# richarddurbin/modimizer

Hardware: AMD Instinct MI355X
Metric: Gbp/s hashed+sketched (k=21,d=64) (higher is better)
Workload: dtype u64; 1 GPU; BASELINE config 2: 10 Gbp synthetic ONT-like reads (log-normal N50 20 kb, 5% subs, 30x of a 333 Mbp genome), k=21 d=64 seed=17, seqhash scan + modset build (table bits 30); reads_per_gpu=598835, bases_per_gpu=10000000000, modimizers_per_gpu=156043826, modset_entries=102967436, k=21, d=64, table_bits=30, parallelism=reads sharded x1, modset per GPU

## Files before the change

modimizer_amd/csrc/mg_common.h:

```cpp
#ifndef MG_COMMON_H
#define MG_COMMON_H
#include "mg_knobs.h"

#include <hip/hip_runtime.h>
#include <stdint.h>
#include <time.h>
#include <algorithm>
#include <vector>
#include "modgpu.h"

#define MG_WAVE 64

#define MG_SCAN_THREADS   256
#define MG_POS_PER_THREAD 64
#define MG_TILE_BASES     (64 * MG_POS_PER_THREAD)
#define MG_TILE_WORDS     (MG_TILE_BASES / 16)

struct MgHashParams {
  U64 factor1;
  U64 mask;
  int k;
  int shift1;
  U32 d;
  int dShift;
// ... 110 lines not shown
#define MG_MIX_MUL 0x9E3779B1u
__device__ __forceinline__ U64 mgMixK (U64 x, int b)
{
  if (b < 24) return mgMixBits (x, b);
  const int lb = b - MG_MIX_TOP;
  const U64 L = x & (((U64) 1 << lb) - 1), A = x >> lb;
  const U32 low = lb >= 32 ? (U32) L : ((U32) L & (((U32) 1 << lb) - 1));
  const U32 g = (low * MG_MIX_MUL) >> (32 - MG_MIX_TOP);
  return ((A ^ (U64) g) << lb) | mgMixBits (L, lb);
}
__device__ __forceinline__ U32 mgMixTopOfKmer (U64 x, int b, int hiB)
{
  const int lb = b - MG_MIX_TOP;
  const U32 low = lb >= 32 ? (U32) x : ((U32) x & (((U32) 1 << lb) - 1));
  return (U32) (x >> (b - hiB)) ^ ((low * MG_MIX_MUL) >> (32 - hiB));
}
__device__ __forceinline__ U32 mgBucketOfM (U64 m, const MgGeom &g)
{
  if (!g.log2NB) return 0u;
  const int s = g.kbits - g.log2NB;
  return s >= 0 ? (U32) (m >> s) : ((U32) m << (-s));
}
__device__ __forceinline__ U32 mgHomeOfM (U64 m, const MgGeom &g)
{
  U32 x = (U32) m;
  if (g.kbits >= 24) x ^= (U32) (m >> (g.kbits - MG_MIX_TOP)) * 0x9E5u;
  return __umulhi (x * 0x85EBCA6Bu, g.R);
}
__device__ __forceinline__ U32 mgNextSlot (U32 at, U32 R) { return at + 1 == R ? 0u : at + 1; }
#endif

static inline unsigned mgGrid (U64 n, unsigned per = 256, unsigned cap = 4096)
{ U64 b = (n + per - 1) / per; if (b > cap) b = cap; if (b < 1) b = 1; return (unsigned) b; }
static inline size_t mgAl256 (size_t n) { return (n + 255) & ~(size_t) 255; }
static inline double mgNowS (void) { struct timespec ts; clock_gettime (CLOCK_MONOTONIC, &ts); return ts.tv_sec + 1e-9 * ts.tv_nsec; }

static inline void mgPartSplit (int log2NB, int *hiB, int *loB)
{ if (log2NB <= 9) { *hiB = log2NB; *loB = 0; } else { *loB = log2NB / 2; *hiB = log2NB - *loB; } }

#define MG_HIST_STRIDE 16
struct MgHistReq { int log2NB; int kbits; U32 *binCount; int hiB; };

struct MgSegSrc { const U64 *segKmer; const U64 *segCount; const U64 *segStart; U64 segCap; U32 nSegs; };


MgStatus mgLaunchPack (const U8 *dBases, U64 nBases, U32 *dWords, hipStream_t st);
MgStatus mgLaunchUnpack (const U32 *dWords, U64 nBases, U8 *dBases, hipStream_t st);
MgStatus mgLaunchScan (const MgHashParams &p, const U32 *dPacked, U64 totalBases,
                       const U64 *dReadOffsets, U32 nReads,
                       U64 *dKmer, U32 *dPosF, U32 *dReadId, U64 capacity,
                       U64 *dCount, void *dWork, hipStream_t st, const MgHistReq *hist = 0, MgSegSrc *lazy = 0);

U64      mgScanTiles (U64 totalBases);
size_t   mgScanInfoBytes (U64 totalBases);
MgStatus mgScanPrepare (const U64 *dReadOffsets, U32 nReads, U64 totalBases, void *dInfo, hipStream_t st);
size_t   mgScanRangeWorkBytes (U64 nTilesRange, U64 capacity);
MgStatus mgLaunchSegCompact (const MgSegSrc &src, U64 *dKmer, U64 capacity, const U64 *dCount, hipStream_t st);
MgStatus mgLaunchScanRange (const MgHashParams &p, const U32 *dPacked, U64 totalBases,
                            const U64 *dReadOffsets, U32 nReads, const void *dInfo, U64 tile0, U64 tile1,
                            U64 *dKmer, U32 *dPosF, U32 *dReadId, U64 capacity,
                            U64 *dCount, void *dWork, hipStream_t st, const MgHistReq *hist = 0, MgSegSrc *lazy = 0);

U64      mgIterMaxBases (void);
U64      mgIterSegEntries (void);
MgStatus mgLaunchIterScan (const MgHashParams &p, const U32 *dPacked, U64 totalBases, const U64 *dReadOff,
                           U64 *dSegKmer, U32 *dSegPosF, U64 *out, U64 capEntries, U64 *flag, U64 seq, hipStream_t st);

MgStatus mgLaunchMinimizers (const MgHashParams &p, U32 w, const U32 *dPacked, const U64 *dReadOffsets, U32 nReads,
                             U64 *dHash, U32 *dPosF, U64 *dReadStart, U64 capacity, U64 *totalOut, hipStream_t st);

struct MgSlot { U64 key; U32 ord; U32 cnt; };
struct MgTable {
  MgSlot *slots; U64 nSlots;
  U64 capSlots;
  U32 capNB;
  U32 R; int log2NB;
  int kbits;
  U32 *occ;
  U64 *value;
  U16 *baseDepth;
  bool baseZero;
  U64 *liveHist;
  bool liveHistValid;
  U32 size;
  U32 max;
  U32 syncedMax;
  U64 *counters;
  bool pendingDepth;
  bool dirty;
  U64 *find8;
  U64 find8Cap;
  U64 find8Version, version;
  bool empty;
  U64 *pin;
  int newPct;
  int loadPct;
  int  maxLog2Slots;
  U32  wantR;
  U64  diag[7];
  int  tightPct;
};
MgStatus mgTableAlloc (MgTable *t, U64 slotsWanted, hipStream_t st);
MgStatus mgTableEnsure (MgTable *t, U64 nIncoming, hipStream_t st);
MgStatus mgTableRollback (MgTable *t, hipStream_t st);
MgStatus mgTableClean (MgTable *t, hipStream_t st);
void     mgTableForget (MgTable *t, hipStream_t st);
size_t   mgTableAddScratchBytes (const MgTable *t, U64 n);
bool     mgTableUseBuckets (const MgTable *t, U64 n);
struct MgValueAside { hipStream_t stream; hipEvent_t merged, done; bool launched; };
MgStatus mgTableAdd (MgTable *t, const U64 *dKmer, U64 n, int withDepth, void *scratch, hipStream_t st,
                     const MgHistReq *counted = 0,
                     const MgSegSrc *segSrc = 0,
// ... 31 lines not shown
```

modimizer_amd/csrc/mg_scan.hip:

```cpp
#include <stdlib.h>
#include <atomic>
#include "mg_prefix.h"


__global__ void mgPackKernel (const U8 *__restrict__ bases, U64 nBases, U32 *__restrict__ words, U64 nWords)
{
  U64 i = (U64) blockIdx.x * blockDim.x + threadIdx.x;
  U64 stride = (U64) gridDim.x * blockDim.x;
  const bool aligned = (((uintptr_t) bases) & 15) == 0;
  for ( ; i < nWords ; i += stride)
    { U64 b0 = i * 16;
      U32 w = 0;
      if (b0 + 16 <= nBases && aligned)
        { uint4 v = *reinterpret_cast<const uint4 *> (bases + b0);
          U32 q[4] = { v.x, v.y, v.z, v.w };
#pragma unroll
          for (int j = 0 ; j < 4 ; ++j)
            { U32 x = q[j];
              U32 n = ((x & 3) << 6) | (((x >> 8) & 3) << 4) | (((x >> 16) & 3) << 2) | ((x >> 24) & 3);
              w |= n << (24 - 8 * j);
            }
        }
      else if (b0 < nBases)
        { for (int j = 0 ; j < 16 && b0 + j < nBases ; ++j)
            w |= (U32) (bases[b0 + j] & 3) << (30 - 2 * j);
        }
      words[i] = w;
    }
}

__global__ void mgUnpackKernel (const U32 *__restrict__ words, U64 nBases, U8 *__restrict__ bases)
{
  U64 i = (U64) blockIdx.x * blockDim.x + threadIdx.x;
  U64 stride = (U64) gridDim.x * blockDim.x;
  for ( ; i < nBases ; i += stride)
    bases[i] = (U8) ((words[i >> 4] >> (30 - 2 * (i & 15))) & 3);
}

MgStatus mgLaunchPack (const U8 *dBases, U64 nBases, U32 *dWords, hipStream_t st)
{
  U64 nWords = (U64) mgPackedWords (nBases);
  if (!nWords) return MG_OK;
  U64 blocks = (nWords + 255) / 256; if (blocks > 8192) blocks = 8192;
  MG_LAUNCH (MG_K_PACK, st, mgPackKernel, dim3 ((unsigned) blocks), dim3 (256), 0, st, dBases, nBases, dWords, nWords);
  MG_HIP (hipGetLastError ());
  return MG_OK;
}

MgStatus mgLaunchUnpack (const U32 *dWords, U64 nBases, U8 *dBases, hipStream_t st)
{
  if (!nBases) return MG_OK;
  U64 blocks = (nBases + 255) / 256; if (blocks > 16384) blocks = 16384;
  MG_LAUNCH (MG_K_UNPACK, st, mgUnpackKernel, dim3 ((unsigned) blocks), dim3 (256), 0, st, dWords, nBases, dBases);
  MG_HIP (hipGetLastError ());
  return MG_OK;
}


__device__ __forceinline__ U32 mgReadOf (const U64 *__restrict__ off, U32 lo, U32 hi, U64 p)
{
  while (lo < hi)
    { U32 mid = lo + (hi - lo + 1) / 2;
      if (off[mid] <= p) lo = mid; else hi = mid - 1;
    }
  return lo;
}

struct __attribute__ ((aligned (32))) MgTileInfo { U64 start, end; U32 firstRead, pad0; U64 pad1; };

__global__ void mgTileInfoKernel (const U64 *__restrict__ readOff, U32 nReads, U64 nTiles, U64 totalBases,
                                  MgTileInfo *__restrict__ info)
{
  U64 t = (U64) blockIdx.x * blockDim.x + threadIdx.x;
  if (t > nTiles) return;
  MgTileInfo ti;
  ti.pad0 = 0; ti.pad1 = 0;
  if (t == nTiles) { ti.firstRead = nReads - 1; ti.start = readOff[nReads - 1]; ti.end = totalBases; }
  else
    { U32 r = mgReadOf (readOff, 0, nReads - 1, t * (U64) MG_TILE_BASES);
      ti.firstRead = r; ti.start = readOff[r]; ti.end = readOff[r + 1];
    }
  info[t] = ti;
}


struct MgScanArgs {
  MgHashParams p;
  const U32 *packed; U64 nWordsAlloc; U64 totalBases;
  const U64 *readOff; U32 nReads;
  const MgTileInfo *tileInfo;
  U64 tileBegin, tileLimit;
  U64 tilesPerWorker;
  U64 nWorkers;
  U64 segCap;
  U64 *segKmer; U32 *segPosF; U32 *segRead;
  U64 *blockCount;
  U32 fS, thresh;
  U32 *histCount;
  int histKbits, histHiB;
#ifdef MG_ABLATE
  U32 debug;
#endif
};

__device__ __forceinline__ U64 mgValidMask (const U64 *off, U32 rBase, U32 nReads, int k, U64 p0, U32 rFirst)
{
  U64 valid = 0;
  U32 r = rFirst;
  for (;;)
    { int64_t start = (int64_t) off[r - rBase], end = (int64_t) off[r + 1 - rBase];
      int64_t lo = start > (int64_t) p0 ? start : (int64_t) p0;
      int64_t hi = end - k; if (hi > (int64_t) p0 + 63) hi = (int64_t) p0 + 63;
      if (hi >= lo)
        { int n = (int) (hi - lo + 1);
          U64 m = (n == 64) ? ~0ull : (((1ull << n) - 1) << (int) (lo - (int64_t) p0));
          valid |= m;
        }
      if (end >= (int64_t) p0 + 64 || r + 1 >= nReads) break;
      ++r;
    }
  return valid;
}

__device__ __forceinline__ bool mgTileInside (const MgScanArgs &a, U64 tile) { return (tile + 1) * MG_TILE_WORDS + 8 <= a.nWordsAlloc; }
__device__ __forceinline__ uint4 mgLoadTileWords (const MgScanArgs &a, U64 tile, int tid, bool inside)
{
  U64 g = tile * MG_TILE_WORDS + 4 * (U64) tid;
  uint4 v;
  if (inside || g + 4 <= a.nWordsAlloc) v = *reinterpret_cast<const uint4 *> (a.packed + g);
  else
    { v.x = g     < a.nWordsAlloc ? a.packed[g]     : 0;
      v.y = g + 1 < a.nWordsAlloc ? a.packed[g + 1] : 0;
      v.z = g + 2 < a.nWordsAlloc ? a.packed[g + 2] : 0;
      v.w = 0;
    }
  return v;
}
__device__ __forceinline__ U32 mgLoadTileHalo (const MgScanArgs &a, U64 tile, int lane, bool inside)
{
  U32 h = 0;
  if (lane < 8) { const U64 gh = tile * MG_TILE_WORDS + MG_TILE_WORDS + lane; h = (inside || gh < a.nWordsAlloc) ? a.packed[gh] : 0; }
  return h;
}

__device__ __forceinline__ U64 mgKmerAt (const U32 *sWords, U32 q, int sh1)
{
  int wi = q >> 4, s = 2 * (q & 15);
  U32 x0 = sWords[wi], x1 = sWords[wi + 1], x2 = sWords[wi + 2];
  U64 hi = ((U64) x0 << 32) | x1;
  if (s) hi = (hi << s) | (U64) (x2 >> (32 - s));
  return hi >> sh1;
}

#define MG_MODE_ANY   0
#define MG_MODE_POW2  1
#define MG_MODE_FAST  2
#define MG_MODE_ODD   3
#define MG_MODE_ODD32 4
#define MG_MODE_ANY32 5
#define MG_MODE_COUNT 6
#define MG_LIST_UNROLL 4
#define MG_CAND_CAP   320
#define MG_WAVES      (MG_SCAN_THREADS / 64)
#ifdef MG_ABLATE
#define MG_ABLATE_AND(x) && (x)
#else
#define MG_ABLATE_AND(x)
#endif

#define MG_WAVE_SYNC() do { __builtin_amdgcn_fence (__ATOMIC_RELEASE, "wavefront"); __builtin_amdgcn_wave_barrier (); \
                            __builtin_amdgcn_fence (__ATOMIC_ACQUIRE, "wavefront"); } while (0)

__device__ __forceinline__ void mgScanHistDone (const MgScanArgs &a, U32 *sHist, U32 *sDone, int lane)
{
  U32 before = 0;
  if (lane == 0) before = __hip_atomic_fetch_add (sDone, 1u, __ATOMIC_RELEASE, __HIP_MEMORY_SCOPE_WORKGROUP);
  before = (U32) __builtin_amdgcn_readfirstlane ((int) before);
  if (before != MG_WAVES - 1) return;
  __builtin_amdgcn_fence (__ATOMIC_ACQUIRE, "workgroup");
  const U32 bins = (U32) 1 << a.histHiB;
  for (U32 b = (U32) lane ; b < bins ; b += 64) { const U32 v = sHist[b]; if (v) atomicAdd (&a.histCount[b * MG_HIST_STRIDE], v); }
}

template <int MODE, bool SINGLE, bool WHERE>
__device__ __forceinline__ U64 mgScanWorker (const MgScanArgs &a, const U64 worker, const int lane,
                                             U32 (*sWordsW)[MG_TILE_WORDS + 8], unsigned short *sCand, U64 *sOff, U32 *sHist)
{
  const MgHashParams &p = a.p;
  const int k = p.k, sh1 = p.shift1;
  const U64 f1 = p.factor1;
  const U64 dMask = (U64) (p.d - 1);

  U64 tile = a.tileBegin + worker * a.tilesPerWorker;
  U64 tileEnd = tile + a.tilesPerWorker; if (tileEnd > a.tileLimit) tileEnd = a.tileLimit;
  const U64 segBase = worker * a.segCap;
  U32 found = 0;
  const U32 segCap32 = a.segCap > 0xffffffffull ? 0xffffffffu : (U32) a.segCap;
  U64 *const segK = a.segKmer + segBase;
  uint4 curV = make_uint4 (0, 0, 0, 0); U32 curHalo = 0;
  MgTileInfo ti, tiNext;
  ti.start = ti.end = 0; ti.firstRead = 0; tiNext = ti;
  U32 nextFirstRead = 0;
  if (tile < tileEnd)
    { const bool inside = mgTileInside (a, tile);
      curV = mgLoadTileWords (a, tile, lane, inside);
      curHalo = mgLoadTileHalo (a, tile, lane, inside);
      if (SINGLE) { ti.start = 0; ti.end = a.totalBases; ti.firstRead = 0; }
      else { ti = a.tileInfo[tile]; nextFirstRead = a.tileInfo[tile + 1].firstRead; }
    }

  int buf = 0;
  U32 qCount = 0, qOld = 0;
  while (tile < tileEnd)
    { U32 *sWords = sWordsW[buf]; buf ^= 1;
      *reinterpret_cast<uint4 *> (&sWords[4 * lane]) = curV;
      if (lane < 8) sWords[MG_TILE_WORDS + lane] = curHalo;

      const U64 tile0 = tile * (U64) MG_TILE_BASES;
      const U64 p0 = tile0 + (U64) lane * MG_POS_PER_THREAD;
      U64 valid = 0;
      U32 rFirst = ti.firstRead;
      const bool oneRead = ti.end >= tile0 + MG_TILE_BASES + (U64) k - 1;
      const bool offInLds = !oneRead && nextFirstRead - ti.firstRead + 2 <= 64;
      if (offInLds)
        { const U32 r = ti.firstRead + (U32) lane;
          if (SINGLE) sOff[lane] = lane == 0 ? 0ull : (lane == 1 ? a.totalBases : ~0ull);
          else sOff[lane] = r <= a.nReads ? a.readOff[r] : ~0ull;
        }
      MG_WAVE_SYNC ();
      if (oneRead) valid = ~0ull;
      else if (p0 < a.totalBases)
        { if (offInLds)
            { rFirst = ti.firstRead + mgReadOf (sOff, 0, nextFirstRead - ti.firstRead, p0);
              valid = mgValidMask (sOff, ti.firstRead, a.nReads, k, p0, rFirst);
            }
          else
            { rFirst = mgReadOf (a.readOff, ti.firstRead, nextFirstRead, p0);
              valid = mgValidMask (a.readOff, 0, a.nReads, k, p0, rFirst);
            }
        }

      const U64 nextTile = tile + 1;
      uint4 nextV = make_uint4 (0, 0, 0, 0); U32 nextHalo = 0; U32 nextNextFirst = 0;
      if (nextTile < tileEnd)
        { const bool inside = mgTileInside (a, nextTile);
          nextV = mgLoadTileWords (a, nextTile, lane, inside);
          nextHalo = mgLoadTileHalo (a, nextTile, lane, inside);
          if (SINGLE) tiNext = ti;
          else { tiNext = a.tileInfo[nextTile]; nextNextFirst = a.tileInfo[nextTile + 1].firstRead; }
        }

      U32 w[6];
      { uint2 h = *reinterpret_cast<const uint2 *> (&sWords[4 * lane + 4]);
        w[0] = curV.x; w[1] = curV.y; w[2] = curV.z; w[3] = curV.w; w[4] = h.x; w[5] = h.y;
      }
      U64 cand;
      if (MODE == MG_MODE_FAST)
        {
          U32 fw[6], rw[6];
          const int c2 = 2 * (k - 16);
#pragma unroll
          for (int j = 0 ; j < 5 ; ++j) fw[j] = __builtin_amdgcn_alignbit (w[j], w[j + 1], 32 - c2);
          fw[5] = w[5] << c2;
#pragma unroll
          for (int j = 0 ; j < 6 ; ++j) rw[j] = mgRevComp16 (w[j]);
          const U32 fS = a.fS, thresh = a.thresh;
          U32 acc = 0, candLo = 0;
#pragma unroll
          for (int chunk = 0 ; chunk < 4 ; ++chunk)
            { const U32 f0 = fw[0], f1w = fw[1], r0 = rw[0], r1 = rw[1];
              fw[0] = fw[1]; fw[1] = fw[2]; fw[2] = fw[3]; fw[3] = fw[4]; fw[4] = fw[5];
              rw[0] = rw[1]; rw[1] = rw[2]; rw[2] = rw[3]; rw[3] = rw[4]; rw[4] = rw[5];
#pragma unroll
              for (int tt = 0 ; tt < 16 ; ++tt)
                { U32 xf = __funnelshift_l (f1w, f0, 2 * tt);
                  U32 xr = __funnelshift_r (r0, r1, 2 * tt);
                  U32 hf = xf * fS, hr = xr * fS;
                  U32 mn = hf < hr ? hf : hr;
                  asm ("v_cmp_gt_u32_e32 vcc, %1, %2\n\tv_addc_co_u32_e32 %0, vcc, %0, %0, vcc"
                       : "+v" (acc) : "s" (thresh), "v" (mn) : "vcc");
                }
              if (chunk == 1) { candLo = acc; acc = 0; }
            }
          cand = ((U64) __brev (acc) << 32) | __brev (candLo);
        }
      else
        {
          U32 rw[6];
#pragma unroll
          for (int j = 0 ; j < 6 ; ++j) rw[j] = mgRevComp16 (w[j]);
          const U32 maskLo = (U32) p.mask, maskHi = (U32) (p.mask >> 32);
          U32 acc = 0, hitLo = 0;
#pragma unroll 1
          for (int chunk = 0 ; chunk < 4 ; ++chunk)
            { const U32 f0 = w[0], f1w = w[1], f2 = w[2], r0 = rw[0], r1 = rw[1], r2 = rw[2];
              w[0] = w[1]; w[1] = w[2]; w[2] = w[3]; w[3] = w[4]; w[4] = w[5];
              rw[0] = rw[1]; rw[1] = rw[2]; rw[2] = rw[3]; rw[3] = rw[4]; rw[4] = rw[5];
#pragma unroll
              for (int tt = 0 ; tt < 16 ; ++tt)
                { const U32 wHi = tt ? __builtin_amdgcn_alignbit (f0, f1w, 32 - 2 * tt) : f0;
                  const U32 wLo = tt ? __builtin_amdgcn_alignbit (f1w, f2, 32 - 2 * tt) : f1w;
                  const U32 xLo = tt ? __builtin_amdgcn_alignbit (r1, r0, 2 * tt) : r0;
                  const U32 xHi = tt ? __builtin_amdgcn_alignbit (r2, r1, 2 * tt) : r1;
                  const U64 F = (((U64) wHi << 32) | wLo) >> sh1;
                  const U64 R = ((U64) (xHi & maskHi) << 32) | (xLo & maskLo);
                  U64 hF = (F * f1) >> sh1, hR = (R * f1) >> sh1;
                  U64 h = hF < hR ? hF : hR;
                  bool hit;
                  if (MODE == MG_MODE_POW2)     hit = (h & dMask) == 0;
                  else if (MODE == MG_MODE_ODD) hit = mgDivisibleOdd (h, p);
                  else if (MODE == MG_MODE_ODD32) hit = mgDivisibleOdd32 (h, p);
                  else if (MODE == MG_MODE_ANY32) hit = mgDivisibleAny32 (h, p);
                  else                          hit = mgDivisible (h, p);
                  acc = (acc << 1) | (hit ? 1u : 0u);
                }
              if (chunk == 1) { hitLo = acc; acc = 0; }
            }
          cand = ((U64) __brev (acc) << 32) | __brev (hitLo);
        }
      cand &= valid;

      const U32 cntLo = (U32) __popc ((U32) cand);
      const U32 cnt = cntLo + (U32) __popc ((U32) (cand >> 32));
      const U32 incl = mgWaveInclusiveSum (cnt);
      const U32 nc = (U32) __builtin_amdgcn_readlane ((int) incl, 63);
      const U32 myFirst = incl - cnt;
#ifdef MG_ABLATE
      if (a.debug & 1)
        { tile = nextTile; curV = nextV; curHalo = nextHalo; ti = tiNext; nextFirstRead = nextNextFirst;
          found += nc >> 20;
          continue;
        }
#endif
      constexpr bool wantWhere = WHERE;
      constexpr int LIST_UNROLL = WHERE ? 0 : MG_LIST_UNROLL;
      const bool lastTile = nextTile >= tileEnd;
      const U32 bufTag = (U32) (buf ^ 1) << 12;
      U32 listed = 0;
      do
        { const U32 room = MG_CAND_CAP - qCount;
          const U32 take = nc - listed < room ? nc - listed : room;
          const U32 lo = listed, hi = listed + take;
          if (lo == 0 && hi == nc)
            { unsigned short *pp = sCand + qCount + myFirst;
#pragma unroll
              for (int half = 0 ; half < 2 ; ++half)
                { U32 c = half ? (U32) (cand >> 32) : (U32) cand;
                  const U32 base = bufTag | ((U32) lane * MG_POS_PER_THREAD + 32u * half);
#pragma unroll
                  for (int j = 0 ; j < LIST_UNROLL ; ++j)
                    { if (!c) break;
                      pp[j] = (unsigned short) (base | (U32) __builtin_ctz (c));
                      c &= c - 1;
                    }
                  if (c)
                    { unsigned short *qq = pp + LIST_UNROLL;
                      do { *qq++ = (unsigned short) (base | (U32) __builtin_ctz (c)); c &= c - 1; } while (c);
                    }
                  if (!half) pp += cntLo;
                }
            }
          else if (take && myFirst < hi && myFirst + cnt > lo)
            { U32 o = myFirst - lo;
#pragma unroll
              for (int half = 0 ; half < 2 ; ++half)
                { U32 c = half ? (U32) (cand >> 32) : (U32) cand;
                  const U32 base = bufTag | ((U32) lane * MG_POS_PER_THREAD + 32u * half);
                  while (c)
                    { const U32 t = (U32) __builtin_ctz (c);
                      c &= c - 1;
                      sCand[o < take ? qCount + o : MG_CAND_CAP] = (unsigned short) (base | t);
                      ++o;
                    }
                }
            }
          MG_WAVE_SYNC ();
          qCount += take; listed = hi;
          U32 nEval = qCount & ~63u;
          if (listed == nc && (wantWhere || lastTile || qOld > nEval)) nEval = qCount;
          U32 waveRun = 0;
#pragma unroll 1
          for (U32 i0 = 0 ; i0 < nEval ; i0 += 64)
            { const U32 i = i0 + (U32) lane;
              const U32 e = sCand[i];
              const U32 q = e & (MG_TILE_BASES - 1);
              U64 F = mgKmerAt (sWordsW[(e >> 12) & 1], q, sh1);
              bool surv, fwd;
              { const U64 R = mgRevComp (F, sh1);
                if (MODE == MG_MODE_FAST)
                  {
                    const U64 PF = F * f1, PR = R * f1;
                    const U32 keep = ~((1u << sh1) - 1u);
                    const U64 cF = (PF & 0xffffffff00000000ull) | ((U32) PF & keep), cR = (PR & 0xffffffff00000000ull) | ((U32) PR & keep);
                    fwd = cF < cR;
                    const U32 lowWord = (U32) (fwd ? PF : PR);
                    surv = (lowWord & ((U32) dMask << sh1)) == 0;
                  }
                else
                  { U64 hF = (F * f1) >> sh1, hR = (R * f1) >> sh1;
                    fwd = hF < hR;
                    U64 h = fwd ? hF : hR;
                    if (MODE == MG_MODE_POW2)     surv = (h & dMask) == 0;
                    else if (MODE == MG_MODE_ODD) surv = mgDivisibleOdd (h, p);
                    else if (MODE == MG_MODE_ODD32) surv = mgDivisibleOdd32 (h, p);
                    else if (MODE == MG_MODE_ANY32) surv = mgDivisibleAny32 (h, p);
                    else                          surv = mgDivisible (h, p);
                  }
                if (!fwd) F = R;
              }
              surv = surv && i < nEval MG_ABLATE_AND (!(a.debug & 4));
              const U64 bs = __ballot (surv);
              U32 r = 0;
              if (wantWhere && (!oneRead || a.segRead)) r = (U32) __shfl ((int) rFirst, (int) (q >> 6));
              if (surv)
                { const U32 o = found + waveRun + (U32) __popcll (bs & (((U64) 1 << lane) - 1));
                  const U64 pos = tile0 + q;
                  U64 rs = ti.start;
                  if (!oneRead && wantWhere)
                    { if (offInLds) { while (sOff[r + 1 - ti.firstRead] <= pos) ++r; rs = sOff[r - ti.firstRead]; }
                      else { while (a.readOff[r + 1] <= pos) ++r; rs = a.readOff[r]; }
                    }
                  if (a.histCount) atomicAdd (&sHist[mgMixTopOfKmer (F, a.histKbits, a.histHiB)], 1u);
                  if (o < segCap32 MG_ABLATE_AND (!(a.debug & 2)))
                    { segK[o] = F;
                      if (WHERE && a.segPosF) a.segPosF[segBase + o] = (U32) (pos - rs) | (fwd ? MG_FWD_BIT : 0u);
                      if (WHERE && a.segRead) a.segRead[segBase + o] = r;
                    }
                }
              waveRun += (U32) __popcll (bs);
            }
          found += waveRun;
          const U32 rem = qCount - nEval;
          if (rem && nEval)
            { const U32 v = (U32) lane < rem ? sCand[nEval + lane] : 0u;
              MG_WAVE_SYNC ();
              if ((U32) lane < rem) sCand[lane] = (unsigned short) v;
            }
          if (nEval) MG_WAVE_SYNC ();
          qOld = qOld > nEval ? qOld - nEval : 0;
          qCount = rem;
        }
      while (listed < nc);
      qOld = qCount;
      tile = nextTile;
      curV = nextV; curHalo = nextHalo; ti = tiNext; nextFirstRead = nextNextFirst;
    }
  return found;
}

template <int MODE, bool WHERE>
__global__ __launch_bounds__ (MG_SCAN_THREADS)
void mgScanKernel (const MgScanArgs a)
{
  __shared__ __attribute__ ((aligned (16))) U32 sWordsAll[MG_WAVES][2][MG_TILE_WORDS + 8];
  __shared__ unsigned short sCandAll[MG_WAVES][MG_CAND_CAP + 2];
  __shared__ U64 sOffAll[MG_WAVES][64];
  __shared__ U32 sHist[512]; __shared__ U32 sDone;

  const int lane = threadIdx.x & 63;
  const int wave = __builtin_amdgcn_readfirstlane ((int) (threadIdx.x >> 6));
  const U64 worker = (U64) blockIdx.x * MG_WAVES + wave;
  if (a.histCount)
    { for (U32 b = threadIdx.x ; b < 512 ; b += MG_SCAN_THREADS) sHist[b] = 0;
      if (threadIdx.x == 0) sDone = 0;
      __syncthreads ();
    }
  if (worker >= a.nWorkers) { if (a.histCount) mgScanHistDone (a, sHist, &sDone, lane); return; }
  const U64 found = mgScanWorker<MODE, false, WHERE> (a, worker, lane, sWordsAll[wave], sCandAll[wave], sOffAll[wave], sHist);
  if (lane == 0) a.blockCount[worker] = found;
  if (a.histCount) mgScanHistDone (a, sHist, &sDone, lane);
}

#define MG_ITER_WAVES     8
#define MG_ITER_MAX_TILES 64
struct MgIterOut { U64 *out; U64 capEntries; volatile U64 *flag; U64 seq; };

template <int MODE>
__global__ __launch_bounds__ (MG_ITER_WAVES * 64)
void mgIterScanKernel (const MgScanArgs a, const MgIterOut o)
{
  __shared__ __attribute__ ((aligned (16))) U32 sWordsAll[MG_ITER_WAVES][2][MG_TILE_WORDS + 8];
  __shared__ unsigned short sCandAll[MG_ITER_WAVES][MG_CAND_CAP + 2];
  __shared__ U64 sOffAll[MG_ITER_WAVES][64];
  __shared__ U64 sFound[MG_ITER_WAVES];
  const int lane = threadIdx.x & 63;
  const int wave = __builtin_amdgcn_readfirstlane ((int) (threadIdx.x >> 6));
  U64 found = 0;
  if ((U64) wave < a.nWorkers) found = mgScanWorker<MODE, true, true> (a, (U64) wave, lane, sWordsAll[wave], sCandAll[wave], sOffAll[wave], (U32 *) 0);
  if (lane == 0) sFound[wave] = found;
  __syncthreads ();
  U64 before = 0, total = 0;
#pragma unroll
  for (int w = 0 ; w < MG_ITER_WAVES ; ++w) { const U64 v = sFound[w]; if (w < wave) before += v; total += v; }
  if (total <= o.capEntries)
    { U32 *posOut = reinterpret_cast<U32 *> (o.out + 1 + total);
      const U64 src = (U64) wave * a.segCap;
      for (U64 i = (U64) lane ; i < found ; i += 64)
        { o.out[1 + before + i] = a.segKmer[src + i];
          posOut[before + i] = a.segPosF[src + i];
        }
    }
  if (threadIdx.x == 0) o.out[0] = total;
  __threadfence_system ();
  __syncthreads ();
  if (threadIdx.x == 0) __hip_atomic_store (const_cast<U64 *> (o.flag), o.seq, __ATOMIC_RELEASE, __HIP_MEMORY_SCOPE_SYSTEM);
}

__global__ __launch_bounds__ (1024)
void mgSegScanKernel (const U64 *__restrict__ blockCount, U32 nBlocks, U64 segCap, U64 capacity,
                      U64 *__restrict__ segStart, U64 *__restrict__ dCount)
{
  __shared__ U64 sV[8192 + 1024];
  __shared__ U64 sWaveSum[16], sWaveMax[16];
  const int tid = threadIdx.x, lane = tid & 63, wave = tid >> 6;
  U64 carry = 0, gmx = 0;
  for (U32 base = 0 ; base < nBlocks ; base += 8192)
    {
#pragma unroll
      for (int j = 0 ; j < 8 ; ++j)
        { U32 e = (U32) j * 1024 + tid, b = base + e;
          sV[e + (e >> 3)] = b < nBlocks ? blockCount[b] : 0;
        }
      __syncthreads ();
      U64 c[8], sum = 0, mx = 0;
// ... 68 lines not shown
          for (int j = 0 ; j < 4 ; ++j)
            { const U64 i = i0 + (U64) j * 256 + threadIdx.x;
              if (i >= n) continue;
              if (outKmer) outKmer[dst + i] = km[j];
              if (outPosF) outPosF[dst + i] = pf[j];
              if (outRead) outRead[dst + i] = rd[j];
              if (histBins)
                { MgGeom hg; hg.R = 0; hg.log2NB = histLog2NB; hg.kbits = histKbits;
                  const U32 bucket = mgBucketOfM (mgMixK (km[j], histKbits), hg);
                  atomicAdd (&sH[(bucket >> histShift) & (histBins - 1)], 1u);
                }
            }
        }
    }
  if (histBins)
    { __syncthreads ();
      for (U32 b = threadIdx.x ; b < histBins ; b += 256) if (sH[b]) atomicAdd (&histCount[b * MG_HIST_STRIDE], sH[b]);
    }
}


static inline U64 mgNumTiles (U64 totalBases) { return (totalBases + MG_TILE_BASES - 1) / MG_TILE_BASES; }

struct MgScanGeom { U64 nTiles, tilesPerBlock; U32 nBlocks; U64 segCap; };
#define MG_SCAN_MAX_BLOCKS 49152

static MgScanGeom mgScanGeometryTiles (U64 nTiles, U64 capacity)
{
  MgScanGeom g;
  g.nTiles = nTiles;
  const long gridKnob = mgKnobs ()->scanGrid;
  const long maxBlocks = gridKnob != MG_KNOB_UNSET && gridKnob > 0 ? gridKnob : MG_SCAN_MAX_BLOCKS;
  U64 want = g.nTiles < (U64) maxBlocks ? g.nTiles : (U64) maxBlocks;
  if (gridKnob == MG_KNOB_UNSET || gridKnob <= 0)
    { U64 fewer = g.nTiles / 8; if (fewer < 8192) fewer = 8192;
      if (want > fewer) want = fewer;
    }
  if (!want) want = 1;
  g.tilesPerBlock = (g.nTiles + want - 1) / want; if (!g.tilesPerBlock) g.tilesPerBlock = 1;
  g.nBlocks = (U32) ((g.nTiles + g.tilesPerBlock - 1) / g.tilesPerBlock); if (!g.nBlocks) g.nBlocks = 1;
  U64 share = capacity / g.nBlocks;
  const long slackKnob = mgKnobs ()->segSlack;
  const bool dense = capacity > (g.nTiles * (U64) MG_TILE_BASES) / 16;
  const U64 slack = slackKnob != MG_KNOB_UNSET && slackKnob >= 1 && slackKnob <= 8 ? (U64) slackKnob : 3;
  U64 seg = slack > 1 ? slack * share + 64 : share + share / 8 + 64;
  if (dense && (slackKnob == MG_KNOB_UNSET || slackKnob < 1 || slackKnob > 8)) seg = share + share / 2 + 64;
  U64 most = g.tilesPerBlock * (U64) MG_TILE_BASES;
  g.segCap = seg < most ? seg : most;
  return g;
}


U64 mgScanTiles (U64 totalBases) { return mgNumTiles (totalBases); }
size_t mgScanInfoBytes (U64 totalBases) { return mgAl256 ((mgNumTiles (totalBases) + 2) * sizeof (MgTileInfo)); }

MgStatus mgScanPrepare (const U64 *dReadOffsets, U32 nReads, U64 totalBases, void *dInfo, hipStream_t st)
{
  U64 nTiles = mgNumTiles (totalBases);
  if (!nTiles || !nReads) return MG_OK;
  MG_LAUNCH (MG_K_TILE_FIRST_READ, st, mgTileInfoKernel, dim3 ((unsigned) ((nTiles + 1 + 255) / 256)), dim3 (256), 0, st,
             dReadOffsets, nReads, nTiles, totalBases, (MgTileInfo *) dInfo);
  MG_HIP (hipGetLastError ());
  return MG_OK;
}

size_t mgScanRangeWorkBytes (U64 nTilesRange, U64 capacity)
{
  MgScanGeom g = mgScanGeometryTiles (nTilesRange, capacity);
  size_t segN = (size_t) g.nBlocks * g.segCap;
  return mgAl256 (g.nBlocks * 8) + mgAl256 ((g.nBlocks + 1) * 8) + mgAl256 (segN * 8) + 2 * mgAl256 (segN * 4) + 256;
}

size_t mgScanWorkBytes (U64 totalBases, U32 nReads, U64 capacity)
{
  (void) nReads;
  return mgScanRangeWorkBytes (mgNumTiles (totalBases), capacity) + mgScanInfoBytes (totalBases);
}

static std::atomic<U64> gScanLaunches[3 * MG_MODE_COUNT];
#define MG_SCAN_COUNTED(i) gScanLaunches[i].fetch_add (1, std::memory_order_relaxed)

extern "C" MgStatus mgScanDiag (U64 *out18)
{
  for (int i = 0 ; i < 3 * MG_MODE_COUNT ; ++i) out18[i] = gScanLaunches[i].load (std::memory_order_relaxed);
  return MG_OK;
}

static int mgScanMode (const MgHashParams &p, MgScanArgs *a)
{
  const bool pow2 = (p.dOddInv == 1 && p.dOddLim == ~0ull);
  const int B = p.shift1 + p.dShift;
  const int forceGeneric = mgKnobs ()->scanGeneric == 1;
  a->fS = 0; a->thresh = 0;
  if (pow2 && p.dShift >= 3 && B <= 32 && p.k >= 17 && !forceGeneric)
    { a->fS = (U32) (p.factor1 << (32 - B));
      a->thresh = (U32) 1 << (32 - p.dShift);
      return MG_MODE_FAST;
    }
  if (pow2) return MG_MODE_POW2;
  const bool small = p.small32 && mgKnobs ()->scanDiv64 != 1;
  return p.dShift == 0 ? (small ? MG_MODE_ODD32 : MG_MODE_ODD) : (small ? MG_MODE_ANY32 : MG_MODE_ANY);
}

MgStatus mgLaunchScanRange (const MgHashParams &p, const U32 *dPacked, U64 totalBases,
                            const U64 *dReadOffsets, U32 nReads, const void *dInfo, U64 tile0, U64 tile1,
                            U64 *dKmer, U32 *dPosF, U32 *dReadId, U64 capacity,
                            U64 *dCount, void *dWork, hipStream_t st, const MgHistReq *hist, MgSegSrc *lazy)
{
  if (lazy) { lazy->segKmer = 0; lazy->nSegs = 0; }
  MG_HIP (hipMemsetAsync (dCount, 0, 4 * sizeof (U64), st));
  if (hist && hist->binCount) MG_HIP (hipMemsetAsync (hist->binCount, 0, 512 * MG_HIST_STRIDE * sizeof (U32), st));
  if (tile1 <= tile0 || !nReads) return MG_OK;
  MgScanGeom g = mgScanGeometryTiles (tile1 - tile0, capacity);
  char *wb = (char *) dWork;
  size_t segN = (size_t) g.nBlocks * g.segCap;
  U64 *blockCount = (U64 *) wb;                  wb += mgAl256 (g.nBlocks * 8);
  U64 *segStart = (U64 *) wb;                    wb += mgAl256 ((g.nBlocks + 1) * 8);
  U64 *segKmer = (U64 *) wb;                     wb += mgAl256 (segN * 8);
  U32 *segPosF = (U32 *) wb;                     wb += mgAl256 (segN * 4);
  U32 *segRead = (U32 *) wb;

  MgScanArgs a;
  a.p = p; a.packed = dPacked; a.nWordsAlloc = (U64) mgPackedWords (totalBases); a.totalBases = totalBases;
  a.readOff = dReadOffsets; a.nReads = nReads; a.tileInfo = (const MgTileInfo *) dInfo;
  a.tileBegin = tile0; a.tileLimit = tile1;
  a.tilesPerWorker = g.tilesPerBlock; a.nWorkers = g.nBlocks; a.segCap = g.segCap;
  a.segKmer = segKmer; a.segPosF = dPosF ? segPosF : 0; a.segRead = dReadId ? segRead : 0; a.blockCount = blockCount;
  a.fS = 0; a.thresh = 0;
  int hHiB = 0, hLoB = 0;
  if (hist && hist->binCount)
    { mgPartSplit (hist->log2NB, &hHiB, &hLoB);
      if (hist->hiB > 0 && hist->hiB <= hist->log2NB && hist->hiB <= 9) { hHiB = hist->hiB; hLoB = hist->log2NB - hHiB; }
    }
  const int histEnv = mgKnobs ()->scanHist == 0 ? 0 : 1;
  const bool scanCounts = histEnv && hist && hist->binCount && hist->kbits >= 24 && hHiB >= 1 && hHiB <= MG_MIX_TOP && hLoB + hHiB == hist->log2NB;
  a.histCount = scanCounts ? hist->binCount : 0; a.histKbits = hist ? hist->kbits : 64; a.histHiB = hHiB;
#ifdef MG_ABLATE
  { const long dbg = mgKnobs ()->scanDebug; a.debug = dbg != MG_KNOB_UNSET ? (U32) dbg : 0u; }
#endif
  const unsigned grid = (g.nBlocks + MG_WAVES - 1) / MG_WAVES;
  const int mode = mgScanMode (p, &a);
  const bool where = a.segPosF || a.segRead;
#define MG_SCAN_LAUNCH(M) do { if (where) { MG_SCAN_COUNTED (2 * (M) + 1); MG_LAUNCH (MG_K_SCAN, st, (mgScanKernel<M, true>), dim3 (grid), dim3 (MG_SCAN_THREADS), 0, st, a); } \
                               else       { MG_SCAN_COUNTED (2 * (M));     MG_LAUNCH (MG_K_SCAN, st, (mgScanKernel<M, false>), dim3 (grid), dim3 (MG_SCAN_THREADS), 0, st, a); } } while (0)
  if (mode == MG_MODE_FAST) MG_SCAN_LAUNCH (MG_MODE_FAST); else if (mode == MG_MODE_POW2) MG_SCAN_LAUNCH (MG_MODE_POW2);
  else if (mode == MG_MODE_ODD) MG_SCAN_LAUNCH (MG_MODE_ODD); else if (mode == MG_MODE_ODD32) MG_SCAN_LAUNCH (MG_MODE_ODD32);
  else if (mode == MG_MODE_ANY32) MG_SCAN_LAUNCH (MG_MODE_ANY32); else MG_SCAN_LAUNCH (MG_MODE_ANY);
#undef MG_SCAN_LAUNCH
  MG_HIP (hipGetLastError ());
  MG_LAUNCH (MG_K_SEG_SCAN, st, mgSegScanKernel, dim3 (1), dim3 (1024), 0, st, blockCount, g.nBlocks, g.segCap, capacity, segStart, dCount);
  MG_HIP (hipGetLastError ());
  { int hiB = 0, loB = 0; U32 bins = 0;
    if (hist && hist->binCount && !scanCounts) { mgPartSplit (hist->log2NB, &hiB, &loB); bins = (U32) 1 << hiB; }
    const unsigned cgrid = g.nBlocks < 4096 ? g.nBlocks : 4096;
    if (lazy) { lazy->segKmer = segKmer; lazy->segCount = blockCount; lazy->segStart = segStart; lazy->segCap = g.segCap; lazy->nSegs = g.nBlocks; }
    if (!lazy || bins || dPosF || dReadId)
      MG_LAUNCH (MG_K_SEG_COMPACT, st, mgSegCompactKernel, dim3 (cgrid), dim3 (256), 0, st,
                 segKmer, a.segPosF, a.segRead, g.segCap, g.nBlocks, blockCount, segStart, lazy ? (U64 *) 0 : dKmer, dPosF, dReadId, capacity, dCount,
                 hist ? hist->log2NB : 0, hist ? hist->kbits : 64, loB, bins, hist ? hist->binCount : (U32 *) 0);
  }
  MG_HIP (hipGetLastError ());
  return MG_OK;
}

MgStatus mgLaunchSegCompact (const MgSegSrc &src, U64 *dKmer, U64 capacity, const U64 *dCount, hipStream_t st)
{
  if (!src.nSegs) return MG_OK;
  const unsigned cgrid = src.nSegs < 4096 ? src.nSegs : 4096;
  MG_LAUNCH (MG_K_SEG_COMPACT, st, mgSegCompactKernel, dim3 (cgrid), dim3 (256), 0, st,
             src.segKmer, (const U32 *) 0, (const U32 *) 0, src.segCap, src.nSegs, src.segCount, src.segStart, dKmer, (U32 *) 0, (U32 *) 0, capacity, dCount,
             0, 64, 0, 0u, (U32 *) 0);
  MG_HIP (hipGetLastError ());
  return MG_OK;
}

MgStatus mgLaunchScan (const MgHashParams &p, const U32 *dPacked, U64 totalBases,
                       const U64 *dReadOffsets, U32 nReads,
                       U64 *dKmer, U32 *dPosF, U32 *dReadId, U64 capacity,
                       U64 *dCount, void *dWork, hipStream_t st, const MgHistReq *hist, MgSegSrc *lazy)
{
  const U64 nTiles = mgNumTiles (totalBases);
  char *info = (char *) dWork + mgScanRangeWorkBytes (nTiles, capacity);
  MgStatus s = mgScanPrepare (dReadOffsets, nReads, totalBases, info, st); if (s) return s;
  return mgLaunchScanRange (p, dPacked, totalBases, dReadOffsets, nReads, info, 0, nTiles,
                            dKmer, dPosF, dReadId, capacity, dCount, dWork, st, hist, lazy);
}


U64 mgIterMaxBases (void) { return (U64) MG_ITER_MAX_TILES * MG_TILE_BASES; }
U64 mgIterSegEntries (void) { return (U64) MG_ITER_MAX_TILES * MG_TILE_BASES; }

MgStatus mgLaunchIterScan (const MgHashParams &p, const U32 *dPacked, U64 totalBases, const U64 *dReadOff,
                           U64 *dSegKmer, U32 *dSegPosF, U64 *out, U64 capEntries, U64 *flag, U64 seq, hipStream_t st)
{
  const U64 nTiles = mgNumTiles (totalBases);
  if (!nTiles || nTiles > MG_ITER_MAX_TILES) { mgSetError ("internal: iterator scan of %llu bases", (unsigned long long) totalBases); return MG_ERR_ARG; }
  MgScanArgs a;
  a.p = p; a.packed = dPacked; a.nWordsAlloc = (U64) mgPackedWords (totalBases); a.totalBases = totalBases;
  a.readOff = dReadOff; a.nReads = 1; a.tileInfo = 0;
  a.tileBegin = 0; a.tileLimit = nTiles;
  a.tilesPerWorker = (nTiles + MG_ITER_WAVES - 1) / MG_ITER_WAVES;
  a.nWorkers = (nTiles + a.tilesPerWorker - 1) / a.tilesPerWorker;
  a.segCap = a.tilesPerWorker * (U64) MG_TILE_BASES;
  a.segKmer = dSegKmer; a.segPosF = dSegPosF; a.segRead = 0; a.blockCount = 0;
  a.histCount = 0; a.histKbits = 64; a.histHiB = 0;
#ifdef MG_ABLATE
  a.debug = 0;
#endif
  MgIterOut o; o.out = out; o.capEntries = capEntries; o.flag = flag; o.seq = seq;
  const int mode = mgScanMode (p, &a);
#define MG_ITER_LAUNCH(M) do { MG_SCAN_COUNTED (2 * MG_MODE_COUNT + (M)); hipLaunchKernelGGL (mgIterScanKernel<M>, dim3 (1), dim3 (MG_ITER_WAVES * 64), 0, st, a, o); } while (0)
  if (mode == MG_MODE_FAST) MG_ITER_LAUNCH (MG_MODE_FAST); else if (mode == MG_MODE_POW2) MG_ITER_LAUNCH (MG_MODE_POW2);
  else if (mode == MG_MODE_ODD) MG_ITER_LAUNCH (MG_MODE_ODD); else if (mode == MG_MODE_ODD32) MG_ITER_LAUNCH (MG_MODE_ODD32);
  else if (mode == MG_MODE_ANY32) MG_ITER_LAUNCH (MG_MODE_ANY32); else MG_ITER_LAUNCH (MG_MODE_ANY);
#undef MG_ITER_LAUNCH
  MG_HIP (hipGetLastError ());
  return MG_OK;
}
```

Baseline: 1268 Gbp/s.

## Drop tile-info precompute kernel; locate reads in-scan with wave-parallel search

Removes the separate per-tile read-info kernel and its work buffer. The scan worker now finds the first read of its tile with a wave-cooperative 64-way search and carries read bounds from tile to tile using the offsets already staged in LDS. It also reads some fields directly from the kernarg segment and tunes SGPR limits per specialization to reduce register pressure. This trades one kernel launch and a global table for extra ballots and searches inside the scan loop, and it relies on positions fitting in 32 bits for read starts.

```diff
diff --git a/modimizer_amd/csrc/mg_common.h b/modimizer_amd/csrc/mg_common.h
--- a/modimizer_amd/csrc/mg_common.h
+++ b/modimizer_amd/csrc/mg_common.h
@@ -186,12 +186,10 @@
                        U64 *dCount, void *dWork, hipStream_t st, const MgHistReq *hist = 0, MgSegSrc *lazy = 0);
 
 U64      mgScanTiles (U64 totalBases);
-size_t   mgScanInfoBytes (U64 totalBases);
-MgStatus mgScanPrepare (const U64 *dReadOffsets, U32 nReads, U64 totalBases, void *dInfo, hipStream_t st);
 size_t   mgScanRangeWorkBytes (U64 nTilesRange, U64 capacity);
 MgStatus mgLaunchSegCompact (const MgSegSrc &src, U64 *dKmer, U64 capacity, const U64 *dCount, hipStream_t st);
 MgStatus mgLaunchScanRange (const MgHashParams &p, const U32 *dPacked, U64 totalBases,
-                            const U64 *dReadOffsets, U32 nReads, const void *dInfo, U64 tile0, U64 tile1,
+                            const U64 *dReadOffsets, U32 nReads, U64 tile0, U64 tile1,
                             U64 *dKmer, U32 *dPosF, U32 *dReadId, U64 capacity,
                             U64 *dCount, void *dWork, hipStream_t st, const MgHistReq *hist = 0, MgSegSrc *lazy = 0);
 
diff --git a/modimizer_amd/csrc/mg_scan.hip b/modimizer_amd/csrc/mg_scan.hip
--- a/modimizer_amd/csrc/mg_scan.hip
+++ b/modimizer_amd/csrc/mg_scan.hip
@@ -1,4 +1,5 @@
 #include <stdlib.h>
+#include <stddef.h>
 #include <atomic>
 #include "mg_prefix.h"
 
@@ -66,21 +67,17 @@
   return lo;
 }
 
-struct __attribute__ ((aligned (32))) MgTileInfo { U64 start, end; U32 firstRead, pad0; U64 pad1; };
-
-__global__ void mgTileInfoKernel (const U64 *__restrict__ readOff, U32 nReads, U64 nTiles, U64 totalBases,
-                                  MgTileInfo *__restrict__ info)
-{
-  U64 t = (U64) blockIdx.x * blockDim.x + threadIdx.x;
-  if (t > nTiles) return;
-  MgTileInfo ti;
-  ti.pad0 = 0; ti.pad1 = 0;
-  if (t == nTiles) { ti.firstRead = nReads - 1; ti.start = readOff[nReads - 1]; ti.end = totalBases; }
-  else
-    { U32 r = mgReadOf (readOff, 0, nReads - 1, t * (U64) MG_TILE_BASES);
-      ti.firstRead = r; ti.start = readOff[r]; ti.end = readOff[r + 1];
-    }
-  info[t] = ti;
+__device__ __forceinline__ U32 mgWaveReadOf (const U64 *__restrict__ off, U32 lo, U32 hi, U64 p, int lane)
+{
+  while (lo < hi)
+    { const U32 step = ((hi - lo - 1) >> 6) + 1;
+      const U64 idx = (U64) lo + (U64) (lane + 1) * step;
+      const bool le = idx <= (U64) hi && off[idx] <= p;
+      const U32 c = (U32) __popcll (__ballot (le));
+      lo += c * step;
+      if (hi - lo > step - 1) hi = lo + (step - 1);
+    }
+  return lo;
 }
 
 
@@ -88,7 +85,6 @@
   MgHashParams p;
   const U32 *packed; U64 nWordsAlloc; U64 totalBases;
   const U64 *readOff; U32 nReads;
-  const MgTileInfo *tileInfo;
   U64 tileBegin, tileLimit;
   U64 tilesPerWorker;
   U64 nWorkers;
@@ -171,6 +167,13 @@
 #define MG_WAVE_SYNC() do { __builtin_amdgcn_fence (__ATOMIC_RELEASE, "wavefront"); __builtin_amdgcn_wave_barrier (); \
                             __builtin_amdgcn_fence (__ATOMIC_ACQUIRE, "wavefront"); } while (0)
 
+template <typename T>
+__device__ __forceinline__ T mgKernarg (size_t offset)
+{
+  typedef const char __attribute__ ((address_space (4))) *Bytes;
+  return *(const T __attribute__ ((address_space (4))) *) ((Bytes) __builtin_amdgcn_kernarg_segment_ptr () + offset);
+}
+
 __device__ __forceinline__ void mgScanHistDone (const MgScanArgs &a, U32 *sHist, U32 *sDone, int lane)
 {
   U32 before = 0;
@@ -197,17 +200,24 @@
   U32 found = 0;
   const U32 segCap32 = a.segCap > 0xffffffffull ? 0xffffffffu : (U32) a.segCap;
   U64 *const segK = a.segKmer + segBase;
+  U32 *const segP = WHERE && a.segPosF ? a.segPosF + segBase : (U32 *) 0, *const segR = WHERE && a.segRead ? a.segRead + segBase : (U32 *) 0;
   uint4 curV = make_uint4 (0, 0, 0, 0); U32 curHalo = 0;
-  MgTileInfo ti, tiNext;
-  ti.start = ti.end = 0; ti.firstRead = 0; tiNext = ti;
-  U32 nextFirstRead = 0;
+  U32 rd = 0, rdStart32 = 0; U64 rdEnd = SINGLE ? a.totalBases : 0;
   if (tile < tileEnd)
     { const bool inside = mgTileInside (a, tile);
       curV = mgLoadTileWords (a, tile, lane, inside);
       curHalo = mgLoadTileHalo (a, tile, lane, inside);
-      if (SINGLE) { ti.start = 0; ti.end = a.totalBases; ti.firstRead = 0; }
-      else { ti = a.tileInfo[tile]; nextFirstRead = a.tileInfo[tile + 1].firstRead; }
-    }
+      if (!SINGLE)
+        { rd = mgWaveReadOf (a.readOff, 0, a.nReads - 1, tile * (U64) MG_TILE_BASES, lane);
+          rdStart32 = (U32) a.readOff[rd]; rdEnd = a.readOff[(U64) rd + 1];
+        }
+    }
+  auto carryRead = [&] (U32 nextRd)
+    { if (SINGLE || nextRd == rd) return;
+      if (nextRd - rd + 2 <= 64) { rdStart32 = (U32) sOff[nextRd - rd]; rdEnd = sOff[nextRd - rd + 1]; }
+      else { rdStart32 = (U32) a.readOff[nextRd]; rdEnd = a.readOff[(U64) nextRd + 1]; }
+      rd = nextRd;
+    };
 
   int buf = 0;
   U32 qCount = 0, qOld = 0;
@@ -219,35 +229,41 @@
       const U64 tile0 = tile * (U64) MG_TILE_BASES;
       const U64 p0 = tile0 + (U64) lane * MG_POS_PER_THREAD;
       U64 valid = 0;
-      U32 rFirst = ti.firstRead;
-      const bool oneRead = ti.end >= tile0 + MG_TILE_BASES + (U64) k - 1;
-      const bool offInLds = !oneRead && nextFirstRead - ti.firstRead + 2 <= 64;
-      if (offInLds)
-        { const U32 r = ti.firstRead + (U32) lane;
-          if (SINGLE) sOff[lane] = lane == 0 ? 0ull : (lane == 1 ? a.totalBases : ~0ull);
-          else sOff[lane] = r <= a.nReads ? a.readOff[r] : ~0ull;
-        }
+      U32 rFirst = rd;
+      const U64 nextTile0 = tile0 + MG_TILE_BASES;
+      const bool oneRead = rdEnd >= nextTile0 + (U64) k - 1;
+      U32 nextRd = rd;
+      if (!oneRead)
+        { if (SINGLE) sOff[lane] = lane == 0 ? 0ull : (lane == 1 ? a.totalBases : ~0ull);
+          else
+            { const U32 nReads = mgKernarg<U32> (offsetof (MgScanArgs, nReads));
+              const U64 r = (U64) rd + (U64) lane;
+              const U64 o = r <= nReads ? a.readOff[r] : ~0ull;
+              sOff[lane] = o;
+              const U32 cnt = (U32) __popcll (__ballot (r < nReads && o <= nextTile0));
+              nextRd = cnt <= 63 ? rd + cnt - 1 : mgWaveReadOf (a.readOff, rd + 63, nReads - 1, nextTile0, lane);
+            }
+        }
+      const bool offInLds = !oneRead && nextRd - rd + 2 <= 64;
       MG_WAVE_SYNC ();
       if (oneRead) valid = ~0ull;
       else if (p0 < a.totalBases)
         { if (offInLds)
-            { rFirst = ti.firstRead + mgReadOf (sOff, 0, nextFirstRead - ti.firstRead, p0);
-              valid = mgValidMask (sOff, ti.firstRead, a.nReads, k, p0, rFirst);
+            { rFirst = rd + mgReadOf (sOff, 0, nextRd - rd, p0);
+              valid = mgValidMask (sOff, rd, a.nReads, k, p0, rFirst);
             }
           else
-            { rFirst = mgReadOf (a.readOff, ti.firstRead, nextFirstRead, p0);
+            { rFirst = mgReadOf (a.readOff, rd, nextRd, p0);
               valid = mgValidMask (a.readOff, 0, a.nReads, k, p0, rFirst);
             }
         }
 
       const U64 nextTile = tile + 1;
-      uint4 nextV = make_uint4 (0, 0, 0, 0); U32 nextHalo = 0; U32 nextNextFirst = 0;
+      uint4 nextV = make_uint4 (0, 0, 0, 0); U32 nextHalo = 0;
       if (nextTile < tileEnd)
         { const bool inside = mgTileInside (a, nextTile);
           nextV = mgLoadTileWords (a, nextTile, lane, inside);
           nextHalo = mgLoadTileHalo (a, nextTile, lane, inside);
-          if (SINGLE) tiNext = ti;
-          else { tiNext = a.tileInfo[nextTile]; nextNextFirst = a.tileInfo[nextTile + 1].firstRead; }
         }
 
       U32 w[6];
@@ -327,7 +343,7 @@
       const U32 myFirst = incl - cnt;
 #ifdef MG_ABLATE
       if (a.debug & 1)
-        { tile = nextTile; curV = nextV; curHalo = nextHalo; ti = tiNext; nextFirstRead = nextNextFirst;
+        { tile = nextTile; curV = nextV; curHalo = nextHalo; carryRead (nextRd);
           found += nc >> 20;
           continue;
         }
@@ -411,20 +427,20 @@
               surv = surv && i < nEval MG_ABLATE_AND (!(a.debug & 4));
               const U64 bs = __ballot (surv);
               U32 r = 0;
-              if (wantWhere && (!oneRead || a.segRead)) r = (U32) __shfl ((int) rFirst, (int) (q >> 6));
+              if (wantWhere && (!oneRead || segR)) r = (U32) __shfl ((int) rFirst, (int) (q >> 6));
               if (surv)
                 { const U32 o = found + waveRun + (U32) __popcll (bs & (((U64) 1 << lane) - 1));
                   const U64 pos = tile0 + q;
-                  U64 rs = ti.start;
+                  U32 rs = rdStart32;
                   if (!oneRead && wantWhere)
-                    { if (offInLds) { while (sOff[r + 1 - ti.firstRead] <= pos) ++r; rs = sOff[r - ti.firstRead]; }
-                      else { while (a.readOff[r + 1] <= pos) ++r; rs = a.readOff[r]; }
+                    { if (offInLds) { while (sOff[r + 1 - rd] <= pos) ++r; rs = (U32) sOff[r - rd]; }
+                      else { while (a.readOff[r + 1] <= pos) ++r; rs = (U32) a.readOff[r]; }
                     }
                   if (a.histCount) atomicAdd (&sHist[mgMixTopOfKmer (F, a.histKbits, a.histHiB)], 1u);
                   if (o < segCap32 MG_ABLATE_AND (!(a.debug & 2)))
                     { segK[o] = F;
-                      if (WHERE && a.segPosF) a.segPosF[segBase + o] = (U32) (pos - rs) | (fwd ? MG_FWD_BIT : 0u);
-                      if (WHERE && a.segRead) a.segRead[segBase + o] = r;
+                      if (WHERE && segP) segP[o] = ((U32) pos - rs) | (fwd ? MG_FWD_BIT : 0u);
+                      if (WHERE && segR) segR[o] = r;
                     }
                 }
               waveRun += (U32) __popcll (bs);
@@ -443,14 +459,13 @@
       while (listed < nc);
       qOld = qCount;
       tile = nextTile;
-      curV = nextV; curHalo = nextHalo; ti = tiNext; nextFirstRead = nextNextFirst;
+      curV = nextV; curHalo = nextHalo; carryRead (nextRd);
     }
   return found;
 }
 
 template <int MODE, bool WHERE>
-__global__ __launch_bounds__ (MG_SCAN_THREADS)
-void mgScanKernel (const MgScanArgs a)
+__device__ __forceinline__ void mgScanKernelBody (const MgScanArgs &a)
 {
   __shared__ __attribute__ ((aligned (16))) U32 sWordsAll[MG_WAVES][2][MG_TILE_WORDS + 8];
   __shared__ unsigned short sCandAll[MG_WAVES][MG_CAND_CAP + 2];
@@ -459,7 +474,9 @@
 
   const int lane = threadIdx.x & 63;
   const int wave = __builtin_amdgcn_readfirstlane ((int) (threadIdx.x >> 6));
-  const U64 worker = (U64) blockIdx.x * MG_WAVES + wave;
+  const U64 worker = (U64) (blockIdx.x * MG_WAVES + (U32) wave);
+  U32 slot = blockIdx.x * MG_WAVES + (threadIdx.x >> 6);
+  asm volatile ("" : "+v" (slot));
   if (a.histCount)
     { for (U32 b = threadIdx.x ; b < 512 ; b += MG_SCAN_THREADS) sHist[b] = 0;
       if (threadIdx.x == 0) sDone = 0;
@@ -467,9 +484,17 @@
     }
   if (worker >= a.nWorkers) { if (a.histCount) mgScanHistDone (a, sHist, &sDone, lane); return; }
   const U64 found = mgScanWorker<MODE, false, WHERE> (a, worker, lane, sWordsAll[wave], sCandAll[wave], sOffAll[wave], sHist);
-  if (lane == 0) a.blockCount[worker] = found;
+  if (lane == 0) mgKernarg<U64 *> (offsetof (MgScanArgs, blockCount))[slot] = found;
   if (a.histCount) mgScanHistDone (a, sHist, &sDone, lane);
 }
+
+template <int MODE, bool WHERE>
+__global__ __launch_bounds__ (MG_SCAN_THREADS) __attribute__ ((amdgpu_num_sgpr (102)))
+void mgScanKernel (const MgScanArgs a) { mgScanKernelBody<MODE, WHERE> (a); }
+template <> __global__ __launch_bounds__ (MG_SCAN_THREADS) __attribute__ ((amdgpu_num_sgpr (0)))
+void mgScanKernel<MG_MODE_ANY, true> (const MgScanArgs a) { mgScanKernelBody<MG_MODE_ANY, true> (a); }
+template <> __global__ __launch_bounds__ (MG_SCAN_THREADS) __attribute__ ((amdgpu_num_sgpr (0)))
+void mgScanKernel<MG_MODE_ANY32, true> (const MgScanArgs a) { mgScanKernelBody<MG_MODE_ANY32, true> (a); }
 
 #define MG_ITER_WAVES     8
 #define MG_ITER_MAX_TILES 64
@@ -644,17 +669,6 @@
 
 
 U64 mgScanTiles (U64 totalBases) { return mgNumTiles (totalBases); }
-size_t mgScanInfoBytes (U64 totalBases) { return mgAl256 ((mgNumTiles (totalBases) + 2) * sizeof (MgTileInfo)); }
-
-MgStatus mgScanPrepare (const U64 *dReadOffsets, U32 nReads, U64 totalBases, void *dInfo, hipStream_t st)
-{
-  U64 nTiles = mgNumTiles (totalBases);
-  if (!nTiles || !nReads) return MG_OK;
-  MG_LAUNCH (MG_K_TILE_FIRST_READ, st, mgTileInfoKernel, dim3 ((unsigned) ((nTiles + 1 + 255) / 256)), dim3 (256), 0, st,
-             dReadOffsets, nReads, nTiles, totalBases, (MgTileInfo *) dInfo);
-  MG_HIP (hipGetLastError ());
-  return MG_OK;
-}
 
 size_t mgScanRangeWorkBytes (U64 nTilesRange, U64 capacity)
 {
@@ -666,7 +680,7 @@
 size_t mgScanWorkBytes (U64 totalBases, U32 nReads, U64 capacity)
 {
   (void) nReads;
-  return mgScanRangeWorkBytes (mgNumTiles (totalBases), capacity) + mgScanInfoBytes (totalBases);
+  return mgScanRangeWorkBytes (mgNumTiles (totalBases), capacity);
 }
 
 static std::atomic<U64> gScanLaunches[3 * MG_MODE_COUNT];
@@ -695,7 +709,7 @@
 }
 
 MgStatus mgLaunchScanRange (const MgHashParams &p, const U32 *dPacked, U64 totalBases,
-                            const U64 *dReadOffsets, U32 nReads, const void *dInfo, U64 tile0, U64 tile1,
+                            const U64 *dReadOffsets, U32 nReads, U64 tile0, U64 tile1,
                             U64 *dKmer, U32 *dPosF, U32 *dReadId, U64 capacity,
                             U64 *dCount, void *dWork, hipStream_t st, const MgHistReq *hist, MgSegSrc *lazy)
 {
@@ -714,7 +728,7 @@
 
   MgScanArgs a;
   a.p = p; a.packed = dPacked; a.nWordsAlloc = (U64) mgPackedWords (totalBases); a.totalBases = totalBases;
-  a.readOff = dReadOffsets; a.nReads = nReads; a.tileInfo = (const MgTileInfo *) dInfo;
+  a.readOff = dReadOffsets; a.nReads = nReads;
   a.tileBegin = tile0; a.tileLimit = tile1;
   a.tilesPerWorker = g.tilesPerBlock; a.nWorkers = g.nBlocks; a.segCap = g.segCap;
   a.segKmer = segKmer; a.segPosF = dPosF ? segPosF : 0; a.segRead = dReadId ? segRead : 0; a.blockCount = blockCount;
@@ -771,10 +785,7 @@
                        U64 *dKmer, U32 *dPosF, U32 *dReadId, U64 capacity,
                        U64 *dCount, void *dWork, hipStream_t st, const MgHistReq *hist, MgSegSrc *lazy)
 {
-  const U64 nTiles = mgNumTiles (totalBases);
-  char *info = (char *) dWork + mgScanRangeWorkBytes (nTiles, capacity);
-  MgStatus s = mgScanPrepare (dReadOffsets, nReads, totalBases, info, st); if (s) return s;
-  return mgLaunchScanRange (p, dPacked, totalBases, dReadOffsets, nReads, info, 0, nTiles,
+  return mgLaunchScanRange (p, dPacked, totalBases, dReadOffsets, nReads, 0, mgNumTiles (totalBases),
                             dKmer, dPosF, dReadId, capacity, dCount, dWork, st, hist, lazy);
 }
 
@@ -789,7 +800,7 @@
   if (!nTiles || nTiles > MG_ITER_MAX_TILES) { mgSetError ("internal: iterator scan of %llu bases", (unsigned long long) totalBases); return MG_ERR_ARG; }
   MgScanArgs a;
   a.p = p; a.packed = dPacked; a.nWordsAlloc = (U64) mgPackedWords (totalBases); a.totalBases = totalBases;
-  a.readOff = dReadOff; a.nReads = 1; a.tileInfo = 0;
+  a.readOff = dReadOff; a.nReads = 1;
   a.tileBegin = 0; a.tileLimit = nTiles;
   a.tilesPerWorker = (nTiles + MG_ITER_WAVES - 1) / MG_ITER_WAVES;
   a.nWorkers = (nTiles + a.tilesPerWorker - 1) / a.tilesPerWorker;
```

After: 1278 Gbp/s, median of 5. About the same (+0.7%).
